# UM-Applied-Algorithms-Lab/AWRY

Measured on AMD Instinct MI355X. Metric: k-mer count queries/sec (parallel_count, random 31-mers, index resident in HBM), higher is better.
Workload: dtype u64

## Files before the change

### awry_amd/csrc/kernels.hip.h

```cpp
#pragma once
#include <hip/hip_runtime.h>

#include "alphabet.h"
#include "layout.h"

namespace awry {

__device__ __forceinline__ SeedEntry seed_probe(const SeedEntry* __restrict__ p) {
  const unsigned long long raw = __builtin_nontemporal_load(reinterpret_cast<const unsigned long long*>(p));
  return SeedEntry{(uint32_t)raw, (uint32_t)(raw >> 32)};
}


__device__ __forceinline__ uint64_t slice_mask(int t) {
  uint64_t m = ~0ull >> (63 - (t > 63 ? 63 : (t < 0 ? 0 : t)));
  return t < 0 ? 0ull : m;
}

template <int A>
__device__ __forceinline__ uint64_t slice_pred(const uint64_t* blk, int l, uint32_t code) {
  uint64_t pr = ~0ull;
#pragma unroll
  for (int b = 0; b < (A == NUCLEOTIDE ? 3 : 5); b++) {
    uint64_t x = ((code >> b) & 1u) ? 0ull : ~0ull;
// ... 915 lines not shown
            ep = scnt ? e.sp + scnt - 1u : 0u;
            i = L - k;
            if (scnt == 1u && i > 0) {
              const uint32_t nc = (uint32_t)(w >> (2 * (i - 1))) & 3u;
              if (seed_sym(e) != (int)(nc == 3u ? 5u : nc + 1u)) { sp = 1u; ep = 0u; }
            }
            if (scnt == SEED_CNT_SAT || (ix.seed_pos && scnt == 1u && sp <= ep && i > 0)) i = -1;
            if (TALLY) t_probe++;
          }
          if (!USE_SEED || i < 0) {
            const uint32_t c = (uint32_t)(w >> (2 * (L - 1))) & 3u;
            sp = c == 0 ? cA : (c == 1 ? cC : (c == 2 ? cG : cT));
            ep = (c == 0 ? cC : (c == 1 ? cG : (c == 2 ? cN : cEnd))) - 1;
            i = L - 1;
          }
          steps_done = 0;
          fresh = false;
        } else {
          i--;
          const uint32_t c = (uint32_t)(w >> (2 * i)) & 3u;
          const uint32_t cl = c == 0 ? cA : (c == 1 ? cC : (c == 2 ? cG : cT));
          if (TALLY) {
            const uint32_t nb = ((sp - 1) >> 8) == (ep >> 8) ? 1u : 2u;
            t_step++;
            t_blk += nb;
            if (steps_done >= TALLY_DEEP_STEP) t_deep += nb;
          }
          quad_step(blocks, cl, sp, ep, c, l);
          steps_done++;
        }
        if (sp > ep || i == 0) {
          finished = true;
          out_count = sp > ep ? 0ull : (uint64_t)(ep - sp) + 1ull;
        } else if (VERIFY) {
          const uint32_t cnt = ep - sp + 1u;
          if (verify_now(cnt, i, steps_done, verify_after)) { mode = 1; vj = 0; vhits = 0; }
        }
      } else if (mode == 1) {
        vp = ix.dense_sa[sp + (uint32_t)vj];
        if (TALLY) t_vsa++;
        if (vp >= (uint32_t)i) mode = 2;
        else vj++;
      } else {
        const uint32_t bad = quad_sum(verify_part(ix.text4, (uint64_t)vp - (uint64_t)i, i, 0, l, w));
        if (TALLY) t_vtxt++;
        if (!bad) vhits++;
        vj++;
        mode = 1;
      }
      if (VERIFY && mode == 1 && vj > (int)(ep - sp)) { finished = true; out_count = vhits; }
      if (finished) {
        if (l == t) res = out_count;
        t++;
        fresh = true;
        mode = 0;
        if (t == nvalid) {
          if (l < nvalid) counts[4 * m + l] = res;
          m += nquads;
          have = m < ngroups;
          t = 0;
          nvalid = have ? (int)(n - 4 * m < 4 ? n - 4 * m : 4) : 0;
          wq = wq_next;
          if (USE_SEED && have) { const SeedEntry e0 = seed[((wq >> kshift) & kmask)]; eq = (uint64_t)e0.sp | ((uint64_t)e0.cnt << 32); }
          wq_next = (m + nquads < ngroups && 4 * (m + nquads) + l < n) ? queries[4 * (m + nquads) + l] : 0;
        }
      }
    }
  }
  if (TALLY && l == 0) {
    atomicAdd(&tally[0], (unsigned long long)t_probe);
    atomicAdd(&tally[1], (unsigned long long)t_step);
    atomicAdd(&tally[2], (unsigned long long)t_blk);
    atomicAdd(&tally[5], (unsigned long long)t_deep);
    if (VERIFY) {
      atomicAdd(&tally[3], (unsigned long long)t_vsa);
      atomicAdd(&tally[4], (unsigned long long)t_vtxt);
    }
  }
}

constexpr int VMULTI = 4;
constexpr int LCX_LANE_ROWS = 4;
constexpr int LCX_TAIL_MAX = 16;

struct Nt2Survivors {
  uint64_t* w;
  uint64_t* range;
  uint32_t* q;
  uint32_t* count;
  uint64_t cap;
  uint32_t* lf_count = nullptr;
};

template <bool TALLY, bool VERIFY>
__device__ __forceinline__ unsigned probe_block(const DevIndex& ix, const uint64_t* __restrict__ queries, uint64_t n, int L,
                                                uint64_t* __restrict__ counts, const Nt2Survivors& sv,
                                                unsigned long long* __restrict__ tally) {
  __shared__ unsigned int s_count;
  constexpr int VQ = 192;
  __shared__ uint64_t s_vw[VERIFY ? 4 : 1][VQ];
  __shared__ uint32_t s_vsp[VERIFY ? 4 : 1][VQ];
  __shared__ uint32_t s_vq[VERIFY ? 4 : 1][VQ];
  __shared__ uint8_t s_vn[VERIFY ? 4 : 1][VQ];
  if (threadIdx.x == 0) s_count = 0;
  if (blockIdx.x == 0 && threadIdx.x == 0 && sv.lf_count) *sv.lf_count = 0;
  __syncthreads();
  const int lane = threadIdx.x & 63, wv_id = threadIdx.x >> 6;
  const SeedEntry* __restrict__ seed = ix.seed;
  const int k = ix.seed_k, i0 = L - k, kshift = 2 * (L - k);
  const uint64_t kmask = (1ull << (2 * k)) - 1;
  const uint64_t stride = (uint64_t)gridDim.x * blockDim.x;
  const uint64_t lane_lt = (1ull << lane) - 1;
  const uint64_t region = (uint64_t)blockIdx.x * sv.cap;
  const bool pos = VERIFY && ix.seed_pos;
  const int cx = (int)ix.ctx_extra, clen = SEED_CTX_LEN + cx;
  const bool verify = VERIFY && (i0 >= 3 || (pos && i0 >= 1));
  const bool lcx = VERIFY && ix.lcx_key != nullptr && i0 >= 1;
  int vcount = 0;
  uint32_t t_vsa = 0, t_vtxt = 0, t_lcx = 0;
  auto drain = [&](int base, int cnt) {
    uint64_t w[2];
    uint32_t q[2], sp[2], nc[2], vp[2];
    bool on[2];
#pragma unroll
    for (int h = 0; h < 2; h++) {
      const int s = base + lane + 64 * h;
      on[h] = lane + 64 * h < cnt;
      w[h] = on[h] ? s_vw[VERIFY ? wv_id : 0][s] : 0;
      q[h] = on[h] ? s_vq[VERIFY ? wv_id : 0][s] : 0;
      sp[h] = on[h] ? s_vsp[VERIFY ? wv_id : 0][s] : 0;
      nc[h] = on[h] ? s_vn[VERIFY ? wv_id : 0][s] : 0;
      vp[h] = sp[h];
      if (on[h] && !(nc[h] & 0x80u) && !(pos && nc[h] == 1u)) { vp[h] = ix.dense_sa[sp[h]]; if (TALLY) t_vsa++; }
    }
#pragma unroll
    for (int h = 0; h < 2; h++) {
      if (!on[h]) continue;
      uint64_t value = 0;
      if (nc[h] & 0x80u) {
        const uint64_t want = (w[h] & ((1ull << (2 * i0)) - 1)) << (64 - 2 * i0);
        const uint32_t rows = nc[h] & 0x7Fu;
        const uint64_t* __restrict__ kp = ix.lcx_key + sp[h];
        const uint64_t k0 = kp[0], k1 = kp[1], k2 = rows > 2u ? kp[2] : ~want, k3 = rows > 3u ? kp[3] : ~want;
        const int sh = 64 - 2 * i0;
        value = (((k0 ^ want) >> sh) == 0) + (((k1 ^ want) >> sh) == 0) + (((k2 ^ want) >> sh) == 0) + (((k3 ^ want) >> sh) == 0);
        if (TALLY) t_lcx++;
        counts[q[h]] = value;
        continue;
      }
      for (uint32_t c = 0; c < nc[h]; c++) {
        const uint32_t p = c ? ix.dense_sa[sp[h] + c] : vp[h];
        if (TALLY && c) t_vsa++;
        if (p >= (uint32_t)i0) {
          if (TALLY) t_vtxt++;
          value += verify_part(ix.text4, (uint64_t)p - (uint64_t)i0, i0, 0, 0, w[h]) ? 0ull : 1ull;
        }
      }
      counts[q[h]] = value;
    }
  };
  constexpr int NQ = 4;
  for (uint64_t wbase = (uint64_t)blockIdx.x * blockDim.x + (threadIdx.x & ~63u); wbase < n; wbase += NQ * stride) {
    uint64_t qv[NQ], wv[NQ];
    SeedEntry ev[NQ];
#pragma unroll
    for (int h = 0; h < NQ; h++) {
      qv[h] = wbase + lane + (uint64_t)h * stride;
      wv[h] = qv[h] < n ? queries[qv[h]] : 0;
    }
#pragma unroll
    for (int h = 0; h < NQ; h++) {
      ev[h] = SeedEntry{1u, 0u};
      if (qv[h] < n) ev[h] = seed_probe(seed + ((wv[h] >> kshift) & kmask));
    }
#pragma unroll
    for (int h = 0; h < NQ; h++) {
      const bool valid = qv[h] < n;
      const uint64_t q = qv[h], w = wv[h];
      const SeedEntry e = ev[h];
      const uint32_t cnt = seed_cnt(e);
      bool survivor = false, queued = false, lcx_q = false;
      uint64_t value = 0;
      if (valid) {
        if (cnt == SEED_CNT_SAT) survivor = true;
        else if (cnt == 0u) value = 0;
        else if (i0 == 0) value = cnt;
        else if (cnt == 1u && pos && seed_has_ctx(e) && i0 <= clen) {
          value = (w & ((1ull << (2 * i0)) - 1)) == (seed_full_ctx(e, cx) >> (2 * (clen - i0))) ? 1ull : 0ull;
        } else if (cnt == 1u && pos && seed_has_ctx(e)) {
          queued = ((w >> (2 * (i0 - clen))) & ((1ull << (2 * clen)) - 1)) == seed_full_ctx(e, cx);
        } else if (cnt == 1u) {
          const uint32_t nc = (uint32_t)(w >> (2 * (i0 - 1))) & 3u;
          survivor = seed_sym(e) == (int)(nc == 3u ? 5u : nc + 1u);
          if (verify && survivor) { queued = true; survivor = false; }
        } else if (lcx && !(e.cnt & (SEED_LCX_NONE | SEED_LCX_TAIL)) && cnt <= (uint32_t)LCX_LANE_ROWS) {
          queued = true;
          lcx_q = true;
        } else if (lcx && !(e.cnt & SEED_LCX_NONE)) {
          survivor = true;
        } else if (verify && cnt <= (uint32_t)VMULTI && (int)(3u * cnt) <= i0 + 2) {
          queued = true;
        } else survivor = true;
        if (!queued) counts[q] = value;
      }
      if (VERIFY) {
        const uint64_t qm = __ballot(queued);
        if (qm) {
          if (queued) {
            const int s = vcount + (int)__popcll(qm & lane_lt);
            s_vw[wv_id][s] = w;
            s_vsp[wv_id][s] = cnt == 1u && pos ? seed_position(e, cx) : e.sp;
            s_vq[wv_id][s] = (uint32_t)q;
            s_vn[wv_id][s] = (uint8_t)(cnt | (lcx_q ? 0x80u : 0u));
          }
          vcount += (int)__popcll(qm);
          __builtin_amdgcn_wave_barrier();
          if (vcount >= 128) {
            vcount -= 128;
            drain(vcount, 128);
            __builtin_amdgcn_wave_barrier();
          }
        }
      }
      const uint64_t sm = __ballot(survivor);
      if (sm) {
        unsigned int slot0 = 0;
        if (lane == 0) slot0 = atomicAdd(&s_count, (unsigned int)__popcll(sm));
        slot0 = __shfl(slot0, 0, 64);
        if (survivor) {
          const uint64_t s = region + slot0 + (uint64_t)__popcll(sm & lane_lt);
          sv.w[s] = w;
          sv.range[s] = (uint64_t)e.sp | ((uint64_t)(cnt | (e.cnt & (SEED_LCX_NONE | SEED_LCX_TAIL))) << 32);
          sv.q[s] = (uint32_t)q;
        }
      }
    }
  }
  if (VERIFY && vcount > 0) drain(0, vcount);
  if (TALLY) {
    if (blockIdx.x == 0 && threadIdx.x == 0) atomicAdd(&tally[0], (unsigned long long)n);
    if (VERIFY && (t_vsa | t_vtxt | t_lcx)) {
      atomicAdd(&tally[3], (unsigned long long)t_vsa);
      atomicAdd(&tally[4], (unsigned long long)t_vtxt);
      atomicAdd(&tally[6], (unsigned long long)t_lcx);
    }
  }
  __syncthreads();
  return s_count;
}

template <bool TALLY, bool VERIFY>
__global__ __launch_bounds__(256) void count_nt2_probe_kernel(DevIndex ix, const uint64_t* __restrict__ queries, uint64_t n, int L,
                                                              uint64_t* __restrict__ counts, Nt2Survivors sv,
                                                              unsigned long long* __restrict__ tally) {
  const unsigned ns = probe_block<TALLY, VERIFY>(ix, queries, n, L, counts, sv, tally);
  if (threadIdx.x == 0) sv.count[blockIdx.x] = ns;
}

template <bool TALLY, bool VERIFY>
__device__ __forceinline__ void resume_block_list(const DevIndex& ix, const Nt2Survivors& sv, uint64_t region, uint64_t ns, int L,
                                                  uint64_t* __restrict__ counts, unsigned long long* __restrict__ tally, bool allow_lcx,
                                                  uint64_t r_start, uint64_t r_stride) {
  const int l = threadIdx.x & 3;
  uint64_t r = r_start;
  const uint64_t* __restrict__ blocks = ix.blocks;
  const int k = ix.seed_k;
  const int verify_after = (int)ix.verify_after;
  const bool lcx = VERIFY && ix.lcx_key != nullptr && allow_lcx;
  const uint32_t cA = (uint32_t)ix.prefix_sums[1], cC = (uint32_t)ix.prefix_sums[2], cG = (uint32_t)ix.prefix_sums[3],
                 cN = (uint32_t)ix.prefix_sums[4], cT = (uint32_t)ix.prefix_sums[5], cEnd = (uint32_t)ix.prefix_sums[6];
  bool have = r < ns, fresh = true;
  uint64_t w = 0;
  uint32_t sp = 1, ep = 0, qidx = 0;
  int i = 0, steps_done = 0;
  int mode = 0, vj = 0;
  uint32_t vhits = 0, vp = 0;
  uint32_t ub_a = 0, ub_b = 0;
  const LcxRefs lq{vp, vhits, ub_a, ub_b, vj};
  uint32_t t_step = 0, t_blk = 0, t_vsa = 0, t_vtxt = 0, t_lcx = 0, t_rp = 0;
  uint64_t nx_w = 0, nx_rg = 0;
  uint32_t nx_q = 0;
  if (have) { nx_w = sv.w[region + r]; nx_rg = sv.range[region + r]; nx_q = sv.q[region + r]; }
  while (__any(have)) {
    if (have) {
      bool finished = false;
      uint64_t out_count = 0;
      if (mode == 0) {
        if (fresh) {
          w = nx_w;
          const uint64_t rg = nx_rg;
          qidx = nx_q;
          if (r + r_stride < ns) { nx_w = sv.w[region + r + r_stride]; nx_rg = sv.range[region + r + r_stride]; nx_q = sv.q[region + r + r_stride]; }
          const uint32_t cf = (uint32_t)(rg >> 32), cnt = cf & SEED_CNT_SAT;
          steps_done = 0;
          fresh = false;
          if (qidx == 0xFFFFFFFFu) {
            sp = 1u; ep = 0u; i = 0;
          } else if (cnt == SEED_CNT_SAT) {
            const uint32_t c = (uint32_t)(w >> (2 * (L - 1))) & 3u;
            sp = c == 0 ? cA : (c == 1 ? cC : (c == 2 ? cG : cT));
            ep = (c == 0 ? cC : (c == 1 ? cG : (c == 2 ? cN : cEnd))) - 1;
            i = L - 1;
          } else {
            sp = (uint32_t)rg;
            ep = sp + cnt - 1u;
            i = L - k;
            if (lcx && cnt >= 2u && !(cf & SEED_LCX_NONE) && i > 0) {
              steps_done = 0;
              if (cf & SEED_LCX_TAIL) mode = 3;
              else { vp = ub_a = sp; vhits = ub_b = sp + cnt; vj = lcx_top_level(sp, cnt); mode = 4; }
            }
          }
        }
        if (mode == 0) {
          const bool skip_step = VERIFY && i > 0 && sp <= ep && verify_now(ep - sp + 1u, i, steps_done, verify_after);
          if (i > 0 && sp <= ep && !skip_step) {
            i--;
            const uint32_t c = (uint32_t)(w >> (2 * i)) & 3u;
            const uint32_t cl = c == 0 ? cA : (c == 1 ? cC : (c == 2 ? cG : cT));
            if (TALLY) { t_step++; t_blk += ((sp - 1) >> 8) == (ep >> 8) ? 1u : 2u; }
            quad_step(blocks, cl, sp, ep, c, l);
            steps_done++;
          }
          if (sp > ep || i == 0) {
            finished = true;
            out_count = sp > ep ? 0ull : (uint64_t)(ep - sp) + 1ull;
          } else if (VERIFY) {
            const uint32_t cnt = ep - sp + 1u;
            if (verify_now(cnt, i, steps_done, verify_after)) { mode = 1; vj = 0; vhits = 0; }
          }
        }
      } else if (mode == 1) {
        vp = ix.dense_sa[sp + (uint32_t)vj];
        if (TALLY) t_vsa++;
        if (vp >= (uint32_t)i) mode = 2;
        else vj++;
      } else if (mode == 2) {
        const uint32_t bad = quad_sum(verify_part(ix.text4, (uint64_t)vp - (uint64_t)i, i, 0, l, w));
        if (TALLY) t_vtxt++;
        if (!bad) vhits++;
        vj++;
        mode = 1;
      } else if (mode == 3) {
        const uint32_t inc = (uint32_t)ix.lcx_key[ep];
        if (TALLY) t_lcx++;
        if (inc > (uint32_t)LCX_TAIL_MAX) { mode = 0; steps_done = 0; }
        else {
          const uint32_t nc = ep - sp + 1u - inc;
          steps_done = (int)inc;
          vp = ub_a = sp; vhits = ub_b = sp + nc; vj = nc ? lcx_top_level(sp, nc) : -1;
          mode = 4;
        }
      } else if (mode == 4) {
        uint64_t qlo, qhi;
        lcx_thresholds(w, i, &qlo, &qhi);
        const int lines = lcx_quad_step(ix, lq, qlo, qhi, l);
        if (TALLY) t_lcx += (uint32_t)lines;
        if (vj < 0) {
          vhits = ub_a - vp;
          if (steps_done) { mode = 5; vj = 0; }
          else { finished = true; out_count = vhits; }
        }
      } else if (mode == 5) {
        vp = (uint32_t)ix.lcx_rowpos[ep + 1u - (uint32_t)steps_done + (uint32_t)vj];
        if (TALLY) t_rp++;
        if (vp >= (uint32_t)i) mode = 6;
        else vj++;
      } else {
        const uint32_t bad = quad_sum(verify_part(ix.text4, (uint64_t)vp - (uint64_t)i, i, 0, l, w));
        if (TALLY) t_vtxt++;
        if (!bad) vhits++;
        vj++;
        mode = 5;
      }
      if (VERIFY && mode == 1 && vj > (int)(ep - sp)) { finished = true; out_count = vhits; }
      if (mode == 5 && vj >= steps_done) { finished = true; out_count = vhits; }
      if (finished) {
        if (l == 0 && qidx != 0xFFFFFFFFu) counts[qidx] = out_count;
        r += r_stride;
        have = r < ns;
        fresh = true;
        mode = 0;
      }
    }
  }
  if (TALLY && l == 0) {
    atomicAdd(&tally[1], (unsigned long long)t_step);
    atomicAdd(&tally[2], (unsigned long long)t_blk);
    if (VERIFY) {
      atomicAdd(&tally[3], (unsigned long long)t_vsa);
      atomicAdd(&tally[4], (unsigned long long)t_vtxt);
      atomicAdd(&tally[6], (unsigned long long)t_lcx);
      atomicAdd(&tally[7], (unsigned long long)t_rp);
    }
  }
}

template <bool TALLY, bool VERIFY>
__global__ __launch_bounds__(256) void count_nt2_resume_kernel(DevIndex ix, Nt2Survivors sv, int L, uint64_t* __restrict__ counts,
                                                               unsigned long long* __restrict__ tally) {
  resume_block_list<TALLY, VERIFY>(ix, sv, (uint64_t)blockIdx.x * sv.cap, (uint64_t)sv.count[blockIdx.x], L, counts, tally, true, threadIdx.x >> 2, 64);
}

template <bool TALLY, bool VERIFY>
__global__ __launch_bounds__(256) void count_nt2_probe_resume_kernel(DevIndex ix, const uint64_t* __restrict__ queries, uint64_t n, int L, uint64_t* __restrict__ counts,
                                   Nt2Survivors sv, unsigned long long* __restrict__ tally) {
  const unsigned ns = probe_block<TALLY, VERIFY>(ix, queries, n, L, counts, sv, tally);
  resume_block_list<TALLY, VERIFY>(ix, sv, (uint64_t)blockIdx.x * sv.cap, (uint64_t)ns, L, counts, tally, true, threadIdx.x >> 2, 64);
}
constexpr int NT2_CHUNK = 256;

template <bool USE_SEED, bool TALLY>
__global__ __launch_bounds__(256) void count_nt2_chunk_kernel(DevIndex ix, const uint64_t* __restrict__ queries, uint64_t n, int L,
                                                              uint64_t* __restrict__ counts, unsigned long long* __restrict__ chunk_counter,
                                                              unsigned long long* __restrict__ tally) {
  __shared__ uint64_t lds_all[4 * NT2_CHUNK];
  const int lane = threadIdx.x & 63, l = lane & 3;
  volatile uint64_t* lds = lds_all + (threadIdx.x >> 6) * NT2_CHUNK;
  const uint64_t* __restrict__ blocks = ix.blocks;
  const SeedEntry* __restrict__ seed = ix.seed;
  const int k = USE_SEED ? ix.seed_k : 1;
  const uint32_t cA = (uint32_t)ix.prefix_sums[1], cC = (uint32_t)ix.prefix_sums[2], cG = (uint32_t)ix.prefix_sums[3],
                 cN = (uint32_t)ix.prefix_sums[4], cT = (uint32_t)ix.prefix_sums[5], cEnd = (uint32_t)ix.prefix_sums[6];
  const uint64_t nchunks = (n + NT2_CHUNK - 1) / NT2_CHUNK;
  const uint64_t quad_lt = (1ull << (lane & ~3)) - 1;
  uint32_t t_probe = 0, t_step = 0, t_blk = 0;

  for (;;) {
    unsigned long long c = 0;
    if (lane == 0) c = atomicAdd(chunk_counter, 1ull);
    c = __shfl(c, 0, 64);
    if (c >= nchunks) break;
    const uint64_t base = c * NT2_CHUNK;
    const int cn = (int)(n - base < (uint64_t)NT2_CHUNK ? n - base : (uint64_t)NT2_CHUNK);
    for (int j = 0; j < NT2_CHUNK / 64; j++) {
      const int s = j * 64 + lane;
      lds[s] = s < cn ? queries[base + s] : 0ull;
    }
    int cursor = 0;
    bool have = false, fresh = true;
    int slot = 0, i = 0;
    uint64_t w = 0;
    uint32_t sp = 1, ep = 0;
    for (;;) {
      const uint64_t needy = __ballot(!have && l == 0);
      if (!have) {
        const int idx = cursor + (int)__popcll(needy & quad_lt);
        if (idx < cn) { have = true; fresh = true; slot = idx; w = lds[idx]; }
      }
      cursor += (int)__popcll(needy);
      if (!__any(have)) break;
      if (have) {
        if (fresh) {
          if (USE_SEED) {
            const uint64_t sidx = ((w >> (2 * (L - k))) & ((1ull << (2 * k)) - 1));
            const SeedEntry e = seed[sidx];
            const uint32_t scnt = seed_cnt(e);
            sp = scnt ? e.sp : 1u;
            ep = scnt ? e.sp + scnt - 1u : 0u;
            i = L - k;
            if (scnt == 1u && i > 0) {
              const uint32_t nc = (uint32_t)(w >> (2 * (i - 1))) & 3u;
              if (seed_sym(e) != (int)(nc == 3u ? 5u : nc + 1u)) { sp = 1u; ep = 0u; }
            }
            if (scnt == SEED_CNT_SAT || (ix.seed_pos && scnt == 1u && sp <= ep && i > 0)) i = -1;
            if (TALLY) t_probe++;
          }
          if (!USE_SEED || i < 0) {
            const uint32_t ch = (uint32_t)(w >> (2 * (L - 1))) & 3u;
            sp = ch == 0 ? cA : (ch == 1 ? cC : (ch == 2 ? cG : cT));
            ep = (ch == 0 ? cC : (ch == 1 ? cG : (ch == 2 ? cN : cEnd))) - 1;
            i = L - 1;
          }
          fresh = false;
        } else {
          i--;
          const uint32_t ch = (uint32_t)(w >> (2 * i)) & 3u;
          const uint32_t cl = ch == 0 ? cA : (ch == 1 ? cC : (ch == 2 ? cG : cT));
          if (TALLY) { t_step++; t_blk += ((sp - 1) >> 8) == (ep >> 8) ? 1u : 2u; }
          quad_step(blocks, cl, sp, ep, ch, l);
        }
        if (sp > ep || i == 0) {
          if (l == 0) lds[slot] = sp > ep ? 0ull : (uint64_t)(ep - sp) + 1ull;
          have = false;
        }
      }
    }
    for (int j = 0; j < NT2_CHUNK / 64; j++) {
      const int s = j * 64 + lane;
      if (s < cn) counts[base + s] = lds[s];
    }
// ... 1265 lines not shown
```

### awry_amd/csrc/launchers.h

```cpp
#pragma once

namespace {

std::atomic<int> g_count_kernel{-1};
int count_kernel_override() {
  int m = g_count_kernel.load();
  if (m >= 0) return m;
  const char* e = getenv("AWRY_COUNT_KERNEL");
  if (e && !strcmp(e, "strided")) return 0;
  if (e && !strcmp(e, "chunk")) return 1;
  if (e && !strcmp(e, "quad4")) return 2;
  if (e && !strcmp(e, "twophase")) return 3;
  return -1;
}
int count_kernel_mode(uint64_t bwt_len, int seed_k, bool seeded) {
  const int m = count_kernel_override();
  if (m >= 0) return m;
  if (seeded && seed_k >= 1 && seed_k <= 31 && (1ull << (2 * seed_k)) / 3 >= bwt_len) return 3;
  return 2;
}


uint64_t list_slots_per_block(uint64_t n, unsigned nblk) { return ((n + (uint64_t)nblk * 256 - 1) / ((uint64_t)nblk * 256)) * 256; }

void launch_pack_nt2(Replica& r, const uint8_t* d_ascii, const uint64_t* d_off, uint64_t base, uint64_t n, uint64_t total_bytes, int L, int W,
                     uint64_t* d_words, uint32_t* d_lens, unsigned long long* d_bad, hipStream_t s, uint32_t* d_bad_list = nullptr) {
  if (n == 0) return;
  const dim3 g(grid_for(r, (n + 63) / 64 * 64, 256)), b(256);
  with_flags(d_off != nullptr, [&](auto R) {
    hipLaunchKernelGGL(pack_nt2_tile_kernel<R()>, g, b, 0, s, d_ascii, d_off, base, n, total_bytes, L, W, d_words, d_lens, d_bad, d_bad_list);
  });
  HIP_CHECK(hipGetLastError());
}

void launch_aa_two_phase(Replica& r, const uint8_t* d_q, const uint64_t* d_off, uint64_t n, int L, uint64_t* d_counts, uint64_t* d_ranges,
                         uint8_t* d_status, hipStream_t s, unsigned long long* d_tally) {
  const ScratchLock scratch_lock(r, s);
  Replica::SurvScratch* sc = surv_scratch(r, s);
  const unsigned nblk = (unsigned)r.num_cus * 8;
  const uint64_t per_block = list_slots_per_block(n, nblk);
  if (sc->cap_q < per_block * nblk) {
    HIP_CHECK(hipStreamSynchronize(s));
    sc->q.alloc(per_block * nblk);
    sc->cap_q = per_block * nblk;
    sc->cap = 0;
  }
  if (!sc->count.p) sc->count.alloc(nblk);
  const bool pooled = nblk <= (unsigned)LIST_MAX_LISTS;
  const QueryList ql{sc->q.p, sc->count.p, per_block, nullptr, nullptr, 0, d_tally, pooled ? nblk : 0u};
  const unsigned nblk2 = pooled ? (unsigned)r.num_cus * 3 : nblk;
  static const bool no_long = getenv("AWRY_AA_LONG") && !strcmp(getenv("AWRY_AA_LONG"), "0");
  const bool lng = d_off ? !no_long : L > AA_KMER_MAX;
  with_flags(d_off != nullptr, lng, [&](auto R, auto G) {
    hipLaunchKernelGGL((count_aa_kmer_probe_kernel<2, R(), G()>), dim3(nblk), dim3(256), 0, s, r.dev, d_q, d_off, n, d_off ? 0 : L, d_counts, d_ranges, d_status, ql);
  });
  hipLaunchKernelGGL((count_scalar_kernel<AMINO, LIST_BLOCK>), dim3(nblk2), dim3(256), 0, s, r.dev, d_q, d_off, n, d_counts, d_ranges, d_status, 1,
                     d_off ? 0 : (uint64_t)L, ql);
  HIP_CHECK(hipGetLastError());
}

void launch_count_ascii(Replica& r, const uint8_t* d_q, const uint64_t* d_off, uint64_t n, uint64_t* d_counts,
                        uint64_t* d_ranges, uint8_t* d_status, hipStream_t s, bool allow_verify, uint64_t ulen = 0, int ref_kmer_len = -1) {
  if (n == 0) return;
  const int vmode = ref_kmer_len >= 0 ? (2 | (ref_kmer_len << 8)) : (allow_verify ? 1 : 0);
  if (ref_kmer_len >= 0) allow_verify = false;
  static const bool aa_off = getenv("AWRY_AA_KMER") && !strcmp(getenv("AWRY_AA_KMER"), "0");
  if (r.dev.alphabet == AMINO && allow_verify && !ulen && d_off && r.seed_k >= 1 && n >= 4096 && n < (1ull << 32) && !aa_off) {
    launch_aa_two_phase(r, d_q, d_off, n, 0, d_counts, d_ranges, d_status, s, nullptr);
    return;
  }
  const dim3 g(grid_for(r, n, 256)), b(256);
  const QueryList none{};
  with_alphabet(r.dev.alphabet, [&](auto A) {
    hipLaunchKernelGGL((count_scalar_kernel<A(), LIST_NONE>), g, b, 0, s, r.dev, d_q, d_off, n, d_counts, d_ranges, d_status, vmode, ulen, none);
  });
  HIP_CHECK(hipGetLastError());
}

uint64_t scan_tiles(uint64_t n) { return (n + SCAN_TILE - 1) / SCAN_TILE; }

void launch_scan(Replica& r, const uint64_t* d_counts, uint64_t n, uint64_t* d_hit_off, uint64_t* d_scratch, hipStream_t s) {
  if (n == 0) { HIP_CHECK(hipMemsetAsync(d_hit_off, 0, 8, s)); return; }
  const uint64_t tiles = scan_tiles(n);
  hipLaunchKernelGGL(scan_tile_sums_kernel, dim3((unsigned)tiles), dim3(256), 0, s, d_counts, n, d_scratch);
  hipLaunchKernelGGL(scan_tile_offsets_kernel, dim3(1), dim3(256), 0, s, d_scratch, tiles, d_scratch + tiles);
  hipLaunchKernelGGL(scan_apply_kernel, dim3((unsigned)tiles), dim3(256), 0, s, d_counts, n, d_scratch, d_hit_off);
  HIP_CHECK(hipGetLastError());
}

void launch_locate(Replica& r, const uint64_t* d_range_start, int rs_stride, const uint64_t* d_hit_off, uint64_t n, uint64_t total,
                   uint64_t* d_gpos, uint64_t* d_pos, hipStream_t s, unsigned long long* d_tally = nullptr) {
  if (total == 0) return;
  unsigned long long* ctr = next_counter(r, s);
  const uint64_t tiles = (total + LOC_TILE - 1) / LOC_TILE;
  const dim3 g((unsigned)std::min<uint64_t>(tiles, (uint64_t)r.num_cus * 8)), b(256);
  const uint32_t run_len = (uint32_t)std::min<uint64_t>(16, std::max<uint64_t>(1, tiles / ((uint64_t)g.x * 4)));
  const uint32_t* dense = r.dense_ratio ? r.dense_sa.p : nullptr;
  with_alphabet(r.dev.alphabet, [&](auto A) {
    hipLaunchKernelGGL(locate_tile_kernel<A()>, g, b, 0, s, r.dev, d_range_start, rs_stride, d_hit_off, n, total, dense, r.dense_ratio, d_gpos, d_pos, ctr, run_len);
  });
  HIP_CHECK(hipGetLastError());
  if (r.dense_ratio == 1) return;
  unsigned long long* wctr = next_counter(r, s);
  if (r.dev.alphabet == NUCLEOTIDE)
    with_flags(d_tally != nullptr, [&](auto T) {
      hipLaunchKernelGGL((locate_walk_nt_lane_kernel<true, T()>), dim3(grid_for(r, total, 256, 4)), b, 0, s, r.dev, total, dense, r.dense_ratio, d_gpos, wctr, d_tally);
    });
  else hipLaunchKernelGGL(locate_walk_kernel<AMINO>, dim3(grid_for(r, total, 256, 7)), b, 0, s, r.dev, total, dense, r.dense_ratio, d_gpos, d_pos, wctr);
  if (d_pos) hipLaunchKernelGGL(localise_walked_kernel, dim3(grid_for(r, total, 256)), b, 0, s, r.dev, total, d_gpos, d_pos);
  HIP_CHECK(hipGetLastError());
}

bool lcx_lanes(const Replica& r) {
  return r.dev.lcx_key != nullptr && r.dev.text4 != nullptr && r.dev.dense_ratio == 1;
}
bool wide_two_phase(uint64_t n) { const int m = count_kernel_override(); return m >= 3 && m <= 5 && n < (1ull << 32); }
uint64_t lcx_lf_list_bound(uint64_t total, unsigned grid) {
  const uint64_t per = (uint64_t)LCX_LF_CHUNK - 15, nwaves = 4ull * grid;
  return total + (total + per - 1) / per * 15 + nwaves * (uint64_t)LCX_LF_CHUNK;
}
void two_phase_lists(Replica& r, hipStream_t s, uint64_t n, unsigned nblk, unsigned lcx_grid, Nt2Survivors* in, Nt2Survivors* out) {
  Replica::SurvScratch* sc = surv_scratch(r, s);
  const uint64_t per_block = list_slots_per_block(n, nblk), total = per_block * nblk;
  const uint64_t fneed = lcx_grid ? lcx_lf_list_bound(total, lcx_grid) : 0;
  if (sc->cap < total || sc->fcap < fneed) {
    HIP_CHECK(hipStreamSynchronize(s));
    if (sc->cap < total) {
      sc->w.alloc(total); sc->range.alloc(total); sc->q.alloc(total);
      sc->cap = sc->cap_q = total;
    }
    if (sc->fcap < fneed) {
      sc->fw.alloc(fneed); sc->frange.alloc(fneed); sc->fq.alloc(fneed);
      sc->fcap = fneed;
    }
  }
  if (!sc->count.p) sc->count.alloc((size_t)r.num_cus * 8);
  if (lcx_grid && !sc->fcount.p) sc->fcount.alloc(8);
  *in = Nt2Survivors{sc->w.p, sc->range.p, sc->q.p, sc->count.p, per_block};
  *out = Nt2Survivors{};
  if (lcx_grid) {
    *out = Nt2Survivors{sc->fw.p, sc->frange.p, sc->fq.p, sc->fcount.p, sc->fcap};
    in->lf_count = sc->fcount.p;
  }
}
template <class K>
unsigned resident_grid(const Replica& r, K kernel) {
  int per_cu = 0;
  if (hipOccupancyMaxActiveBlocksPerMultiprocessor(&per_cu, kernel, 256, 0) != hipSuccess || per_cu < 1) { (void)hipGetLastError(); per_cu = 2; }
  return (unsigned)r.num_cus * (unsigned)per_cu;
}

void launch_count_nt2_long(Replica& r, const uint64_t* d_words, uint64_t n, int L, uint64_t* d_counts, uint64_t* d_range_start,
                           bool use_seed, hipStream_t s, const uint32_t* d_lens = nullptr) {
  require(r.dev.alphabet == NUCLEOTIDE, "packed 2-bit queries need a nucleotide index");
  require(L >= 1 && L <= 1 << 20, "packed read length out of range");
  if (n == 0) return;
  const ScratchLock scratch_lock(r, s);
  if (r.wide) {
    const bool sdw = use_seed && r.seed_k > 0 && r.dev.seed64 && (d_lens || r.seed_k <= L);
    const dim3 gw(grid_for(r, n * 4, 256)), bw(256);
    if (sdw && wide_two_phase(n)) {
      Nt2Survivors sv, fb;
      const unsigned nblk = (unsigned)r.num_cus * 8;
      two_phase_lists(r, s, n, nblk, 0u, &sv, &fb);
      with_flags(d_lens != nullptr, [&](auto R) {
        hipLaunchKernelGGL((count_nt2_wide_probe_kernel<R(), false>), dim3(nblk), bw, 0, s, r.dev, d_words, n, L, d_counts, d_range_start, sv, d_lens, (unsigned long long*)nullptr);
        hipLaunchKernelGGL((count_nt2_wide_kernel<true, R(), true>), dim3(nblk), bw, 0, s, r.dev, d_words, n, L, d_counts, d_range_start, d_lens, (unsigned long long*)nullptr, sv);
      });
      HIP_CHECK(hipGetLastError());
      return;
    }
    with_flags(sdw, d_lens != nullptr, [&](auto S, auto R) {
      hipLaunchKernelGGL((count_nt2_wide_kernel<S(), R()>), gw, bw, 0, s, r.dev, d_words, n, L, d_counts, d_range_start, d_lens, (unsigned long long*)nullptr);
    });
    HIP_CHECK(hipGetLastError());
    return;
  }
  const bool sd = use_seed && r.seed_k > 0 && (d_lens || r.seed_k <= L);
  const bool vfy = r.dev.text4 && r.dev.dense_ratio == 1;
  const dim3 g(grid_for(r, n * 4, 256)), b(256);
  const int om = count_kernel_override();
  if (vfy && sd && L - r.seed_k >= 3 && L <= 512 && n < (1ull << 32) && (om < 0 || (om >= 3 && om <= 5))) {
    const unsigned nblk = (unsigned)r.num_cus * 8;
    const unsigned gl = r.lcx_reads_grid[d_lens != nullptr];
    const bool lanes = lcx_lanes(r) && gl > 0 && nblk <= (unsigned)LIST_MAX_LISTS && lcx_lf_list_bound(list_slots_per_block(n, nblk) * nblk, gl) <= 0xFFFFFFFFull;
    Nt2Survivors sv, fb;
    two_phase_lists(r, s, n, nblk, lanes ? gl : 0u, &sv, &fb);
    if (!lanes) sv.w = sv.range = nullptr;
    const dim3 gq((unsigned)r.num_cus * 8);
    with_flags(d_lens != nullptr, [&](auto R) {
      hipLaunchKernelGGL(count_nt2_reads_probe_kernel<R()>, dim3(nblk), b, 0, s, r.dev, d_words, n, L, d_counts, d_range_start, sv, d_lens);
      if (lanes) {
        hipLaunchKernelGGL(lcx_quad_reads_kernel<R()>, dim3(gl), b, 0, s, r.dev, d_words, L, d_counts, d_range_start, sv, fb, nblk, d_lens);
        hipLaunchKernelGGL(count_nt2_reads_pool_kernel<R()>, gq, b, 0, s, r.dev, d_words, L, d_counts, d_range_start, fb, d_lens);
      } else hipLaunchKernelGGL((count_nt2_reads_kernel<true, true, true, R()>), dim3(nblk), b, 0, s, r.dev, d_words, n, L, d_counts, d_range_start, sv, d_lens);
    });
    HIP_CHECK(hipGetLastError());
    return;
  }
  const Nt2Survivors none{};
  with_flags(sd, vfy, d_lens != nullptr, [&](auto S, auto V, auto R) {
    hipLaunchKernelGGL((count_nt2_reads_kernel<S(), V(), false, R()>), g, b, 0, s, r.dev, d_words, n, L, d_counts, d_range_start, none, d_lens);
  });
  HIP_CHECK(hipGetLastError());
}

void launch_count_nt2(Replica& r, const uint64_t* d_words, uint64_t n, int L, uint64_t* d_counts, bool use_seed, hipStream_t s,
                      unsigned long long* d_tally = nullptr) {
  require(r.dev.alphabet == NUCLEOTIDE, "packed 2-bit queries need a nucleotide index");
  require(L >= 1 && L <= 32, "packed k-mer length must be in 1..32");
  if (n == 0) return;
  const ScratchLock scratch_lock(r, s);
  if (r.wide) {
    const bool sdw = use_seed && r.seed_k > 0 && r.dev.seed64 && r.seed_k <= L;
    const dim3 gw(grid_for(r, n * 4, 256)), bw(256);
    if (sdw && wide_two_phase(n)) {
      Nt2Survivors sv, fb;
      const unsigned nblk = (unsigned)r.num_cus * 8;
      two_phase_lists(r, s, n, nblk, 0u, &sv, &fb);
// ... 116 lines not shown
```

### awry_amd/csrc/prewarm.h

```cpp
#pragma once

namespace {

void prewarm_host_paths(Replica& r) {
  static const bool off = getenv("AWRY_PREWARM") && !strcmp(getenv("AWRY_PREWARM"), "0");
  if (off) return;
  HIP_CHECK(hipSetDevice(r.device));
  (void)HostPool::instance();
  const bool nt = r.dev.alphabet == NUCLEOTIDE;
  const uint64_t cap = 1u << 20, W = 4;
  std::unique_lock<std::mutex> lane_lock(r.lane_mu);
  size_t free_b = 0, total_b = 0;
  const bool hbm_plenty = hipMemGetInfo(&free_b, &total_b) == hipSuccess && free_b > (32ull << 30);
  if (nt) {
    for (int li = 0; li < Replica::NLANES; li++) {
      PackedLane& ln = prepare_count_lane(r, li, cap);
      ln.h_words.ensure(cap * W);
      ensure(ln.words, cap * W);
    }
    for (int li = 0; li < 2; li++) {
      LocateLane& ln = prepare_locate_lane(r, li, cap, W, 1);
      static const bool big_hits = !(getenv("AWRY_PREWARM_HITS") && !strcmp(getenv("AWRY_PREWARM_HITS"), "0"));
      const uint64_t hits_cap = hbm_plenty && big_hits ? 16 * cap : cap + cap / 4;
      if (ln.gpos.n < hits_cap) ln.gpos.alloc(hits_cap);
      if (ln.pos.n < 2 * hits_cap) ln.pos.alloc(2 * hits_cap);
    }
    for (int li = 0; li < Replica::NLANES; li++) {
      Replica::SurvScratch* sc = surv_scratch(r, r.lane_stream[li]);
      uint64_t total = 0;
      for (const unsigned nblk : {(unsigned)r.num_cus * (unsigned)r.probe_resume_per_cu[1], (unsigned)r.num_cus * 8})
        total = std::max<uint64_t>(total, list_slots_per_block(cap, nblk) * nblk);
      if (sc->cap < total) { sc->w.alloc(total); sc->range.alloc(total); sc->q.alloc(total); sc->cap = sc->cap_q = total; }
      if (!sc->count.p) sc->count.alloc((size_t)r.num_cus * 8);
      if (!sc->counters.p) sc->counters.alloc(8);
    }
  }
  static std::once_flag once;
  void* warm_block = nullptr;
  std::call_once(once, [&] {
    const char* e = getenv("AWRY_PINNED_PREWARM_MB");
    const size_t budget = (size_t)((e && atof(e) >= 0 ? atof(e) : 1024.0) * (double)(1u << 20));
    const size_t sizes[5] = {64u << 20, 64u << 20, 128u << 20, 256u << 20, 512u << 20};
    void* blocks[5] = {nullptr, nullptr, nullptr, nullptr, nullptr};
    size_t used = 0;
    for (int i = 0; i < 5 && used + sizes[i] <= budget; i++) { blocks[i] = PinnedPool::instance().get(sizes[i]); used += sizes[i]; }
    warm_block = blocks[0];
    for (int i = 1; i < 5; i++)
      if (blocks[i]) release_result(blocks[i]);
  });
  static const int lmask = getenv("AWRY_PREWARM_LOCATE") ? atoi(getenv("AWRY_PREWARM_LOCATE")) : 7;
  const bool warm_locate = lmask != 0;
  if (nt && warm_locate && r.dev.bwt_len >= 4)
    for (int li = 0; li < 2; li++) {
      LocateLane& ln = r.loc_lanes[li];
      hipStream_t s = r.lane_stream[li];
      if (lmask & 1) {
        memset(ln.h_words.p, 0, 16 * W * 8);
        HIP_CHECK(hipMemcpyAsync(ln.words.p, ln.h_words.p, 16 * W * 8, hipMemcpyHostToDevice, s));
        HIP_CHECK(hipMemsetAsync(ln.bad.p, 0, 8, s));
        HIP_CHECK(hipMemsetAsync(ln.bad.p + 1, 0xFF, 8, s));
        launch_count_nt2_long(r, ln.words.p, 16, 101, ln.counts.p, ln.rstart.p, true, s, nullptr);
        const QueryList ql{nullptr, nullptr, 0, ln.bad.p, ln.bad.p + 1, 1};
        hipLaunchKernelGGL((count_scalar_kernel<NUCLEOTIDE, LIST_GLOBAL>), dim3(1), dim3(256), 0, s, r.dev, (const uint8_t*)nullptr, (const uint64_t*)nullptr,
                           (uint64_t)0, ln.counts.p, ln.rstart.p, nullptr, 1, (uint64_t)101, ql);
        HIP_CHECK(hipGetLastError());
      }
      if (lmask & 2) {
        ln.h_meta.p[0] = r.dev.bwt_len / 2;
        ln.h_meta.p[1] = 1;
        HIP_CHECK(hipMemcpyAsync(ln.rstart.p, ln.h_meta.p, 8, hipMemcpyHostToDevice, s));
        HIP_CHECK(hipMemcpyAsync(ln.counts.p, ln.h_meta.p + 1, 8, hipMemcpyHostToDevice, s));
        launch_scan(r, ln.counts.p, 1, ln.hit_off.p, ln.scratch.p, s);
        launch_locate(r, ln.rstart.p, 1, ln.hit_off.p, 1, 1, ln.gpos.p, ln.pos.p, s);
        HIP_CHECK(hipMemcpyAsync(ln.h_meta.p, ln.hit_off.p + 1, 8, hipMemcpyDeviceToHost, s));
      }
      if (warm_block && (lmask & 4)) {
        HIP_CHECK(hipMemcpyAsync(warm_block, ln.gpos.p, cap * 8, hipMemcpyDeviceToHost, s));
        HIP_CHECK(hipMemcpyAsync(static_cast<char*>(warm_block) + cap * 8, ln.pos.p, cap * 16, hipMemcpyDeviceToHost, s));
      }
      HIP_CHECK(hipEventRecord(ln.located, s));
      HIP_CHECK(hipEventSynchronize(ln.located));
      HIP_CHECK(hipStreamSynchronize(s));
    }
  if (warm_block) release_result(warm_block);
  if (nt)
    for (int li = 0; li < Replica::NLANES; li++) {
      PackedLane& ln = r.lanes[li];
      hipStream_t s = r.lane_stream[li];
      memset(ln.h_words.p, 0, cap * 8);
      const auto c0 = std::chrono::steady_clock::now();
      HIP_CHECK(hipMemcpyAsync(ln.words.p, ln.h_words.p, cap * 8, hipMemcpyHostToDevice, s));
      if (getenv("AWRY_TRACE_HOST"))
        fprintf(stderr, "[awry] warm-up, count lane %d: enqueue of the chunk-sized copy in took %.2f ms\n", li,
                std::chrono::duration<double, std::milli>(std::chrono::steady_clock::now() - c0).count());
      launch_count_nt2(r, ln.words.p, 64, r.seed_k > 0 && r.seed_k < 31 ? r.seed_k + 1 : 31, ln.counts.p, true, s, nullptr);
      launch_count_nt2_long(r, ln.words.p, 16, 101, ln.counts.p, nullptr, true, s, nullptr);
      hipLaunchKernelGGL(narrow_counts_kernel, dim3(grid_for(r, cap, 1024)), dim3(256), 0, s, ln.counts.p, ln.counts32.p, cap);
      HIP_CHECK(hipMemcpyAsync(ln.h_counts32.p, ln.counts32.p, cap * 4, hipMemcpyDeviceToHost, s));
      HIP_CHECK(hipEventRecord(ln.done, s));
      HIP_CHECK(hipEventSynchronize(ln.done));
      HIP_CHECK(hipStreamSynchronize(s));
    }
  lane_lock.unlock();
  if (nt && !r.wide && !(getenv("AWRY_PREWARM_REALCOUNT") && !strcmp(getenv("AWRY_PREWARM_REALCOUNT"), "0"))) {
    const uint64_t n = 3ull << 20;
    std::vector<uint64_t> words(n, 0), counts(n, 0);
    PackedPlan plan;
    plan.ok = true;
    plan.Lmax = 31;
    count_shard_hostpacked(r, nullptr, nullptr, Shard{0, n}, plan, counts.data(), words.data());
  }
}

}
```

Measured before the change: 39.12 billion.

## Add lane-per-query LCX search stage splitting survivors into two per-block lists

Survivors whose seed entry has an LCX tree and a short remaining suffix are now written to the front of each block's survivor region. The rest are written backwards from the end. A new lcx_lane_stage processes the front list one query per lane, using quad-cooperative DPP broadcasts to load 16 keys per level and a popcount-based range narrowing, followed by tail position/text verification. The remaining survivors go through the existing 4-lane resume path, which now reads its list downward from the top. The aim is to cut the per-query lane waste and divergence of the quad-based resume for LCX lookups, at the cost of an extra stage, more register pressure and a doubled count array.

```diff
diff --git a/awry_amd/csrc/kernels.hip.h b/awry_amd/csrc/kernels.hip.h
--- a/awry_amd/csrc/kernels.hip.h
+++ b/awry_amd/csrc/kernels.hip.h
@@ -1021,6 +1021,7 @@
 constexpr int VMULTI = 4;
 constexpr int LCX_LANE_ROWS = 4;
 constexpr int LCX_TAIL_MAX = 16;
+constexpr int LCX_LANE_MAX_I = 16;
 
 struct Nt2Survivors {
   uint64_t* w;
@@ -1031,17 +1032,18 @@
   uint32_t* lf_count = nullptr;
 };
 
+struct Nt2ListLens { unsigned lanes, quads; };
 template <bool TALLY, bool VERIFY>
-__device__ __forceinline__ unsigned probe_block(const DevIndex& ix, const uint64_t* __restrict__ queries, uint64_t n, int L,
+__device__ __forceinline__ Nt2ListLens probe_block(const DevIndex& ix, const uint64_t* __restrict__ queries, uint64_t n, int L,
                                                 uint64_t* __restrict__ counts, const Nt2Survivors& sv,
                                                 unsigned long long* __restrict__ tally) {
-  __shared__ unsigned int s_count;
+  __shared__ unsigned int s_count, s_back;
   constexpr int VQ = 192;
   __shared__ uint64_t s_vw[VERIFY ? 4 : 1][VQ];
   __shared__ uint32_t s_vsp[VERIFY ? 4 : 1][VQ];
   __shared__ uint32_t s_vq[VERIFY ? 4 : 1][VQ];
   __shared__ uint8_t s_vn[VERIFY ? 4 : 1][VQ];
-  if (threadIdx.x == 0) s_count = 0;
+  if (threadIdx.x == 0) s_count = s_back = 0;
   if (blockIdx.x == 0 && threadIdx.x == 0 && sv.lf_count) *sv.lf_count = 0;
   __syncthreads();
   const int lane = threadIdx.x & 63, wv_id = threadIdx.x >> 6;
@@ -1055,6 +1057,7 @@
   const int cx = (int)ix.ctx_extra, clen = SEED_CTX_LEN + cx;
   const bool verify = VERIFY && (i0 >= 3 || (pos && i0 >= 1));
   const bool lcx = VERIFY && ix.lcx_key != nullptr && i0 >= 1;
+  const bool lane_search = lcx && i0 <= LCX_LANE_MAX_I;
   int vcount = 0;
   uint32_t t_vsa = 0, t_vtxt = 0, t_lcx = 0;
   auto drain = [&](int base, int cnt) {
@@ -1118,7 +1121,7 @@
       const uint64_t q = qv[h], w = wv[h];
       const SeedEntry e = ev[h];
       const uint32_t cnt = seed_cnt(e);
-      bool survivor = false, queued = false, lcx_q = false;
+      bool survivor = false, queued = false, lcx_q = false, to_lane = false;
       uint64_t value = 0;
       if (valid) {
         if (cnt == SEED_CNT_SAT) survivor = true;
@@ -1137,6 +1140,7 @@
           lcx_q = true;
         } else if (lcx && !(e.cnt & SEED_LCX_NONE)) {
           survivor = true;
+          to_lane = lane_search;
         } else if (verify && cnt <= (uint32_t)VMULTI && (int)(3u * cnt) <= i0 + 2) {
           queued = true;
         } else survivor = true;
@@ -1163,11 +1167,17 @@
       }
       const uint64_t sm = __ballot(survivor);
       if (sm) {
-        unsigned int slot0 = 0;
-        if (lane == 0) slot0 = atomicAdd(&s_count, (unsigned int)__popcll(sm));
+        const uint64_t lm = __ballot(to_lane), bm = sm & ~lm;
+        unsigned int slot0 = 0, slot1 = 0;
+        if (lane == 0) {
+          if (lm) slot0 = atomicAdd(&s_count, (unsigned int)__popcll(lm));
+          if (bm) slot1 = atomicAdd(&s_back, (unsigned int)__popcll(bm));
+        }
         slot0 = __shfl(slot0, 0, 64);
+        slot1 = __shfl(slot1, 0, 64);
         if (survivor) {
-          const uint64_t s = region + slot0 + (uint64_t)__popcll(sm & lane_lt);
+          const uint64_t s = to_lane ? region + slot0 + (uint64_t)__popcll(lm & lane_lt)
+                                     : region + sv.cap - 1u - slot1 - (uint64_t)__popcll(bm & lane_lt);
           sv.w[s] = w;
           sv.range[s] = (uint64_t)e.sp | ((uint64_t)(cnt | (e.cnt & (SEED_LCX_NONE | SEED_LCX_TAIL))) << 32);
           sv.q[s] = (uint32_t)q;
@@ -1185,19 +1195,24 @@
     }
   }
   __syncthreads();
-  return s_count;
+  return Nt2ListLens{s_count, s_back};
 }
 
 template <bool TALLY, bool VERIFY>
 __global__ __launch_bounds__(256) void count_nt2_probe_kernel(DevIndex ix, const uint64_t* __restrict__ queries, uint64_t n, int L,
                                                               uint64_t* __restrict__ counts, Nt2Survivors sv,
                                                               unsigned long long* __restrict__ tally) {
-  const unsigned ns = probe_block<TALLY, VERIFY>(ix, queries, n, L, counts, sv, tally);
-  if (threadIdx.x == 0) sv.count[blockIdx.x] = ns;
-}
+  const Nt2ListLens ns = probe_block<TALLY, VERIFY>(ix, queries, n, L, counts, sv, tally);
+  if (threadIdx.x == 0) { sv.count[blockIdx.x] = ns.lanes; sv.count[gridDim.x + blockIdx.x] = ns.quads; }
+}
+
+}
+#include "lcx_lane.hip.h"
+namespace awry {
+
 
 template <bool TALLY, bool VERIFY>
-__device__ __forceinline__ void resume_block_list(const DevIndex& ix, const Nt2Survivors& sv, uint64_t region, uint64_t ns, int L,
+__device__ __forceinline__ void resume_block_list(const DevIndex& ix, const Nt2Survivors& sv, uint64_t top, uint64_t ns, int L,
                                                   uint64_t* __restrict__ counts, unsigned long long* __restrict__ tally, bool allow_lcx,
                                                   uint64_t r_start, uint64_t r_stride) {
   const int l = threadIdx.x & 3;
@@ -1219,7 +1234,7 @@
   uint32_t t_step = 0, t_blk = 0, t_vsa = 0, t_vtxt = 0, t_lcx = 0, t_rp = 0;
   uint64_t nx_w = 0, nx_rg = 0;
   uint32_t nx_q = 0;
-  if (have) { nx_w = sv.w[region + r]; nx_rg = sv.range[region + r]; nx_q = sv.q[region + r]; }
+  if (have) { nx_w = sv.w[top - r]; nx_rg = sv.range[top - r]; nx_q = sv.q[top - r]; }
   while (__any(have)) {
     if (have) {
       bool finished = false;
@@ -1229,7 +1244,7 @@
           w = nx_w;
           const uint64_t rg = nx_rg;
           qidx = nx_q;
-          if (r + r_stride < ns) { nx_w = sv.w[region + r + r_stride]; nx_rg = sv.range[region + r + r_stride]; nx_q = sv.q[region + r + r_stride]; }
+          if (r + r_stride < ns) { nx_w = sv.w[top - r - r_stride]; nx_rg = sv.range[top - r - r_stride]; nx_q = sv.q[top - r - r_stride]; }
           const uint32_t cf = (uint32_t)(rg >> 32), cnt = cf & SEED_CNT_SAT;
           steps_done = 0;
           fresh = false;
@@ -1338,14 +1353,18 @@
 template <bool TALLY, bool VERIFY>
 __global__ __launch_bounds__(256) void count_nt2_resume_kernel(DevIndex ix, Nt2Survivors sv, int L, uint64_t* __restrict__ counts,
                                                                unsigned long long* __restrict__ tally) {
-  resume_block_list<TALLY, VERIFY>(ix, sv, (uint64_t)blockIdx.x * sv.cap, (uint64_t)sv.count[blockIdx.x], L, counts, tally, true, threadIdx.x >> 2, 64);
+  const uint64_t region = (uint64_t)blockIdx.x * sv.cap;
+  lcx_lane_stage<TALLY>(ix, sv, region, sv.count[blockIdx.x], L, counts, tally);
+  resume_block_list<TALLY, VERIFY>(ix, sv, region + sv.cap - 1u, (uint64_t)sv.count[gridDim.x + blockIdx.x], L, counts, tally, true, threadIdx.x >> 2, 64);
 }
 
 template <bool TALLY, bool VERIFY>
 __global__ __launch_bounds__(256) void count_nt2_probe_resume_kernel(DevIndex ix, const uint64_t* __restrict__ queries, uint64_t n, int L, uint64_t* __restrict__ counts,
                                    Nt2Survivors sv, unsigned long long* __restrict__ tally) {
-  const unsigned ns = probe_block<TALLY, VERIFY>(ix, queries, n, L, counts, sv, tally);
-  resume_block_list<TALLY, VERIFY>(ix, sv, (uint64_t)blockIdx.x * sv.cap, (uint64_t)ns, L, counts, tally, true, threadIdx.x >> 2, 64);
+  const Nt2ListLens ns = probe_block<TALLY, VERIFY>(ix, queries, n, L, counts, sv, tally);
+  const uint64_t region = (uint64_t)blockIdx.x * sv.cap;
+  lcx_lane_stage<TALLY>(ix, sv, region, ns.lanes, L, counts, tally);
+  resume_block_list<TALLY, VERIFY>(ix, sv, region + sv.cap - 1u, (uint64_t)ns.quads, L, counts, tally, true, threadIdx.x >> 2, 64);
 }
 constexpr int NT2_CHUNK = 256;
 
diff --git a/awry_amd/csrc/launchers.h b/awry_amd/csrc/launchers.h
--- a/awry_amd/csrc/launchers.h
+++ b/awry_amd/csrc/launchers.h
@@ -45,7 +45,7 @@
     sc->cap_q = per_block * nblk;
     sc->cap = 0;
   }
-  if (!sc->count.p) sc->count.alloc(nblk);
+  if (!sc->count.p) sc->count.alloc((size_t)r.num_cus * 16);
   const bool pooled = nblk <= (unsigned)LIST_MAX_LISTS;
   const QueryList ql{sc->q.p, sc->count.p, per_block, nullptr, nullptr, 0, d_tally, pooled ? nblk : 0u};
   const unsigned nblk2 = pooled ? (unsigned)r.num_cus * 3 : nblk;
@@ -134,7 +134,7 @@
       sc->fcap = fneed;
     }
   }
-  if (!sc->count.p) sc->count.alloc((size_t)r.num_cus * 8);
+  if (!sc->count.p) sc->count.alloc((size_t)r.num_cus * 16);
   if (lcx_grid && !sc->fcount.p) sc->fcount.alloc(8);
   *in = Nt2Survivors{sc->w.p, sc->range.p, sc->q.p, sc->count.p, per_block};
   *out = Nt2Survivors{};
diff --git a/awry_amd/csrc/lcx_lane.hip.h b/awry_amd/csrc/lcx_lane.hip.h
--- /dev/null
+++ b/awry_amd/csrc/lcx_lane.hip.h
@@ -0,0 +1,183 @@
+#pragma once
+
+namespace awry {
+
+__device__ __forceinline__ int lcx_lane_level(uint32_t a, uint32_t b) {
+  return a ? (31 - __clz((int)((a - 1u) ^ (b - 1u)))) >> 2 : 7;
+}
+
+template <int J>
+__device__ __forceinline__ uint32_t quad_bcast(uint32_t v) {
+  return (uint32_t)__builtin_amdgcn_mov_dpp((int)v, J * 0x55, 0xF, 0xF, true);
+}
+
+template <bool TALLY>
+__device__ __forceinline__ void lcx_lane_stage(const DevIndex& ix, const Nt2Survivors& sv, uint64_t region, uint32_t ne, int L,
+                                               uint64_t* __restrict__ counts, unsigned long long* __restrict__ tally) {
+  enum : int { M_FETCH = 0, M_TAILCNT, M_SEARCH, M_POS, M_TXT };
+  const int i = L - ix.seed_k;
+  const uint32_t cmask = i >= 16 ? ~0u : (1u << (2 * i)) - 1u;
+  const int qsh = 32 - 2 * i;
+  const uint32_t qfill = i >= 16 ? 0u : (1u << qsh) - 1u;
+  const uint64_t wmask = i >= 16 ? ~0ull : (1ull << (4 * i)) - 1ull;
+  const uint32_t* __restrict__ key32 = reinterpret_cast<const uint32_t*>(ix.lcx_key);
+  const uint32_t* __restrict__ inner32 = reinterpret_cast<const uint32_t*>(ix.lcx_inner);
+  const uint32_t* __restrict__ rowpos32 = reinterpret_cast<const uint32_t*>(ix.lcx_rowpos);
+  const uint32_t* __restrict__ wlo32 = reinterpret_cast<const uint32_t*>(sv.w + region);
+  const uint64_t* __restrict__ rangep = sv.range + region;
+  const uint32_t* __restrict__ qp = sv.q + region;
+  __shared__ unsigned int s_next;
+  if (threadIdx.x == 0) s_next = blockDim.x;
+  __syncthreads();
+  const uint64_t lane_lt = (1ull << (threadIdx.x & 63)) - 1;
+  uint32_t r = threadIdx.x;
+  bool have = r < ne;
+  int mode = M_FETCH;
+  uint32_t ctx = 0, qidx = 0;
+  uint32_t a0 = 0, b0 = 0, a1 = 0, b1 = 0;
+  uint32_t inc = 0, tb = 0, vj = 0, vp = 0;
+  uint32_t t_lcx = 0, t_rp = 0, t_vtxt = 0;
+  const int l = threadIdx.x & 3;
+  uint32_t K[16];
+  uint32_t D[4];
+#pragma unroll
+  for (int e = 0; e < 16; e++) K[e] = 0;
+#pragma unroll
+  for (int e = 0; e < 4; e++) D[e] = 0;
+  while (__any(have)) {
+    int s = 0;
+    uint32_t j0 = 0, jh0 = 0, j1 = 0, jh1 = 0, nd = 0;
+    bool up0 = false, up1 = false;
+    const bool srch = have && mode == M_SEARCH;
+    uint32_t plo = 0, phi = 0;
+    if (have) {
+      const uint32_t* p = wlo32 + 2ull * r;
+      if (mode == M_TAILCNT) p = key32 + 2ull * (b0 - 1u);
+      if (mode == M_POS) p = rowpos32 + 2ull * (tb + vj);
+      if (mode == M_TXT) p = ix.text4 + ((vp - (uint32_t)i) >> 3);
+      if (mode == M_SEARCH) {
+        const int l0 = a0 < b0 ? lcx_lane_level(a0, b0) : -1, l1 = a1 < b1 ? lcx_lane_level(a1, b1) : -1;
+        const int t = l0 > l1 ? l0 : l1;
+        s = 4 * t;
+        j0 = ((a0 - 1u) >> s) + 1u; jh0 = (b0 - 1u) >> s;
+        j1 = ((a1 - 1u) >> s) + 1u; jh1 = (b1 - 1u) >> s;
+        if (a0 == 0u) j0 = 0u;
+        if (a1 == 0u) j1 = 0u;
+        up0 = l0 == t;
+        nd = (up0 ? j0 : j1) & ~15u;
+        up1 = l1 == t && (j1 & ~15u) == nd;
+        uint32_t off = 0;
+#pragma unroll
+        for (int u = 1; u < 8; u++) off = t == u ? ix.lcx_off[u] : off;
+        p = (t == 0 ? key32 : inner32 + 2ull * off) + 2ull * nd + 1;
+      }
+      plo = (uint32_t)(uintptr_t)p; phi = (uint32_t)((uintptr_t)p >> 32);
+      if (mode != M_SEARCH) D[0] = p[0];
+      if (mode == M_FETCH) {
+        const uint64_t rg = rangep[r];
+        D[1] = (uint32_t)rg; D[2] = (uint32_t)(rg >> 32);
+        D[3] = qp[r];
+      }
+      if (mode == M_TXT) { D[1] = p[1]; D[2] = p[2]; }
+    }
+    const uint32_t srch_bit = srch ? 1u : 0u;
+    const uint32_t f0 = quad_bcast<0>(srch_bit), f1 = quad_bcast<1>(srch_bit), f2 = quad_bcast<2>(srch_bit), f3 = quad_bcast<3>(srch_bit);
+#define LCX_LANE_ROUND(J, F)                                                                                                  \
+    if (F) {                                                                                                                  \
+      const uint32_t* pj = reinterpret_cast<const uint32_t*>((uintptr_t)quad_bcast<J>(plo) | ((uintptr_t)quad_bcast<J>(phi) << 32)) + 8 * l; \
+      K[4 * J + 0] = pj[0]; K[4 * J + 1] = pj[2]; K[4 * J + 2] = pj[4]; K[4 * J + 3] = pj[6];                                     \
+    }
+    LCX_LANE_ROUND(0, f0) LCX_LANE_ROUND(1, f1) LCX_LANE_ROUND(2, f2) LCX_LANE_ROUND(3, f3)
+#undef LCX_LANE_ROUND
+    asm volatile("" : "+v"(K[0]), "+v"(K[1]), "+v"(K[2]), "+v"(K[3]), "+v"(K[4]), "+v"(K[5]), "+v"(K[6]), "+v"(K[7]),
+                      "+v"(K[8]), "+v"(K[9]), "+v"(K[10]), "+v"(K[11]), "+v"(K[12]), "+v"(K[13]), "+v"(K[14]), "+v"(K[15]),
+                      "+v"(D[0]), "+v"(D[1]), "+v"(D[2]), "+v"(D[3]));
+    uint32_t lt = 0, le = 0;
+    {
+      const uint32_t qlo = ctx << qsh, qhi = qlo | qfill;
+#define LCX_LANE_ROUND(J, F)                                                                                                  \
+      if (F) {                                                                                                                \
+        const uint32_t qlj = quad_bcast<J>(qlo), qhj = quad_bcast<J>(qhi);                                                     \
+        uint32_t m = 0;                                                                                                       \
+        _Pragma("unroll") for (int u = 0; u < 4; u++)                                                                       \
+          m |= (K[4 * J + u] < qlj ? 1u << u : 0u) | (K[4 * J + u] <= qhj ? 0x10000u << u : 0u);                            \
+        m = quad_sum(m << (4 * l));                                                                      \
+        if (l == J) { lt = m & 0xFFFFu; le = m >> 16; }                                                                       \
+      }
+      LCX_LANE_ROUND(0, f0) LCX_LANE_ROUND(1, f1) LCX_LANE_ROUND(2, f2) LCX_LANE_ROUND(3, f3)
+#undef LCX_LANE_ROUND
+    }
+    bool finished = false;
+    if (have) {
+      if (mode == M_FETCH) {
+        ctx = D[0] & cmask;
+        qidx = D[3];
+        const uint32_t cnt = D[2] & SEED_CNT_SAT;
+        a0 = a1 = D[1];
+        b0 = b1 = D[1] + cnt;
+        inc = 0;
+        mode = (D[2] & SEED_LCX_TAIL) ? M_TAILCNT : M_SEARCH;
+      } else if (mode == M_TAILCNT) {
+        inc = D[0];
+        if (TALLY) t_lcx++;
+        b0 -= inc;
+        b1 = tb = b0;
+        mode = M_SEARCH;
+      } else if (mode == M_SEARCH) {
+        if (TALLY) t_lcx++;
+        if (up0) {
+          const uint32_t hi = jh0 - nd < 15u ? jh0 - nd : 15u;
+          const uint32_t c = (uint32_t)__popc(lt & ((2u << hi) - 1u) & ~((1u << (j0 - nd)) - 1u));
+          if (j0 + c <= jh0) b0 = (j0 + c) << s;
+          if (c) a0 = ((j0 + c - 1u) << s) + 1u;
+        }
+        if (up1) {
+          const uint32_t hi = jh1 - nd < 15u ? jh1 - nd : 15u;
+          const uint32_t c = (uint32_t)__popc(le & ((2u << hi) - 1u) & ~((1u << (j1 - nd)) - 1u));
+          if (j1 + c <= jh1) b1 = (j1 + c) << s;
+          if (c) a1 = ((j1 + c - 1u) << s) + 1u;
+        }
+      } else if (mode == M_POS) {
+        vp = D[0];
+        if (TALLY) t_rp++;
+        if (vp >= (uint32_t)i) mode = M_TXT;
+        else vj++;
+      } else {
+        const int sh = 4 * (int)((vp - (uint32_t)i) & 7u);
+        const uint64_t x = (uint64_t)D[0] | ((uint64_t)D[1] << 32);
+        const uint64_t win = sh ? (x >> sh) | ((uint64_t)D[2] << (64 - sh)) : x;
+        if (TALLY) t_vtxt++;
+        if (((win ^ spread_letters16(ctx)) & wmask) == 0) a1++;
+        vj++;
+        mode = M_POS;
+      }
+      if (mode == M_SEARCH && a0 >= b0 && a1 >= b1) {
+        a1 -= a0;
+        vj = 0;
+        mode = M_POS;
+      }
+      if (mode == M_POS && vj >= inc) finished = true;
+      if (finished) {
+        counts[qidx] = (uint64_t)a1;
+        mode = M_FETCH;
+      }
+    }
+    const uint64_t fm = __ballot(finished);
+    if (fm) {
+      unsigned int base = 0;
+      if ((threadIdx.x & 63) == 0) base = atomicAdd(&s_next, (unsigned int)__popcll(fm));
+      base = __builtin_amdgcn_readfirstlane(base);
+      if (finished) {
+        r = base + (uint32_t)__popcll(fm & lane_lt);
+        have = r < ne;
+      }
+    }
+  }
+  if (TALLY && (t_lcx | t_rp | t_vtxt)) {
+    atomicAdd(&tally[4], (unsigned long long)t_vtxt);
+    atomicAdd(&tally[6], (unsigned long long)t_lcx);
+    atomicAdd(&tally[7], (unsigned long long)t_rp);
+  }
+}
+
+}
diff --git a/awry_amd/csrc/prewarm.h b/awry_amd/csrc/prewarm.h
--- a/awry_amd/csrc/prewarm.h
+++ b/awry_amd/csrc/prewarm.h
@@ -31,7 +31,7 @@
       for (const unsigned nblk : {(unsigned)r.num_cus * (unsigned)r.probe_resume_per_cu[1], (unsigned)r.num_cus * 8})
         total = std::max<uint64_t>(total, list_slots_per_block(cap, nblk) * nblk);
       if (sc->cap < total) { sc->w.alloc(total); sc->range.alloc(total); sc->q.alloc(total); sc->cap = sc->cap_q = total; }
-      if (!sc->count.p) sc->count.alloc((size_t)r.num_cus * 8);
+      if (!sc->count.p) sc->count.alloc((size_t)r.num_cus * 16);
       if (!sc->counters.p) sc->counters.alloc(8);
     }
   }
```

Result: no change. 38.93 billion (-0.5%).
